# Gallicchio-Lab/openmm_agbnp_plugin

Hardware: AMD Instinct MI355X
Metric: AGBNP1 force-eval-limited ns/day (1 fs step), thrombin 1dwc, independent replicas (higher is better)
Workload: dtype f64

## Files before the change

### openmm_agbnp_plugin_amd/AGBNPplugin.py

```python
import ctypes as C

import numpy as np

from . import _lib


class OpenMMException(Exception):
    """Same role as OpenMM::OpenMMException in the reference: every API error surfaces as this type."""


def _md_unit_system():
    for name in ("openmm.unit", "simtk.unit"):
        try:
            module = __import__(name, fromlist=["md_unit_system"])
            return module.md_unit_system
        except Exception:
            continue
    return "md_unit_system"


def _strip_units(value):
    if hasattr(value, "value_in_unit_system"):
        return float(value.value_in_unit_system(_md_unit_system()))
    return float(value)
# ... 183 lines not shown
        if _lib.load().agbnp_hip_poll(self._h, C.byref(done), C.byref(bad)) != _lib.OK:
            raise OpenMMException("agbnp_hip_poll: no pinned status memory")
        return int(done.value), int(bad.value)

    def wait_verdict(self, evaluations=0, timeout=10.0):
        self._need()
        done, bad = C.c_int(0), C.c_int(0)
        rc = _lib.load().agbnp_hip_wait_verdict(self._h, int(evaluations), float(timeout), C.byref(done), C.byref(bad))
        if rc == _lib.ERR_TIMEOUT:
            raise OpenMMException(f"agbnp_hip_wait_verdict: timed out after {timeout} s with {int(done.value)} evaluation(s) judged")
        if rc != _lib.OK:
            raise OpenMMException("agbnp_hip_wait_verdict: no pinned status memory")
        return int(done.value), int(bad.value)

    def withheld(self):
        self._need()
        lib = _lib.load()
        n = lib.agbnp_hip_withheld_evaluations(self._h, None, 0)
        idx = np.full(max(n, 1), -1, dtype=np.int32)
        lib.agbnp_hip_withheld_evaluations(self._h, _ip(idx), n)
        return [int(k) for k in idx if k >= 0]

    def generation(self):
        self._need()
        return int(_lib.load().agbnp_hip_generation(self._h))

    def copyParametersToContext(self, force):
        self._need()
        r, g, a, q, h = force._arrays()
        rc = _lib.load().agbnp_hip_update_parameters(self._h, len(r), _dp(r), _dp(g), _dp(a), _dp(q), _ip(h))
        if rc != _lib.OK:
            raise OpenMMException(_lib.last_error(self._h))

    SCALARS = dict(e_vol1=0, e_vol2=1, e_atom=2, e_gb_pair=3, max_subtree_nodes=4, total_nodes=5, variant=6, max_local_atoms=7, forests=8, rows_on=9, row_builds=10, pack_level=11, pack_age=12, row_slice=13, pack_plans=14, overflow_kinds=15, launches=16, healed_forests=17)
    VECTORS = dict(selfvol_vdw=0, born=1, scale=2, selfvol_large=3, subtree_nodes=4, subtree_atoms=5)

    def scalar(self, name):
        self._need()
        v = C.c_double(0)
        rc = _lib.load().agbnp_hip_get_scalar(self._h, self.SCALARS[name], C.byref(v))
        if rc != _lib.OK:
            raise OpenMMException(_lib.last_error(self._h))
        return v.value

    def vector(self, name):
        self._need()
        out = np.zeros(self.numParticles)
        rc = _lib.load().agbnp_hip_get_vector(self._h, self.VECTORS[name], _dp(out))
        if rc != _lib.OK:
            raise OpenMMException(_lib.last_error(self._h))
        return out

    def tables(self):
        self._need()
        lib = _lib.load()
        ni, nj = C.c_int(0), C.c_int(0)
        lib.agbnp_hip_get_table_sizes(self._h, C.byref(ni), C.byref(nj))
        y = np.zeros(ni.value * nj.value * 16)
        y2 = np.zeros_like(y)
        ti = np.zeros(self.numParticles, dtype=np.int32)
        tj = np.zeros(self.numParticles, dtype=np.int32)
        lib.agbnp_hip_get_tables(self._h, _dp(y), _dp(y2), _ip(ti), _ip(tj))
        return dict(y=y.reshape(ni.value, nj.value, 16), y2=y2.reshape(ni.value, nj.value, 16), type_screened=ti, type_screener=tj)

    def set_diagnostics(self, enabled):
        self._need()
        _lib.load().agbnp_hip_set_diagnostics(self._h, 1 if enabled else 0)
# ... 70 lines not shown
```

### openmm_agbnp_plugin_amd/csrc/engine.hip

```cpp
#include <hip/hip_runtime.h>

#include <algorithm>
#include <atomic>
#include <chrono>
#include <cmath>
#include <cstdio>
#include <cstdlib>
#include <cstring>
#include <string>
#include <vector>

#include "../../include/agbnp_hip.h"
#include "adapter_kernels.h"
#include "agbnp_common.h"
#include "i4_tables.h"
#include "pair_kernels.h"
#include "tree_kernels.h"

namespace agbnp {
size_t tree_variant_lds_bytes(int variant);
size_t tree_variant_scratch_bytes(int variant);
int tree_variant_node_cap(int variant);
int tree_variant_atom_cap(int variant);
int tree_variant_wgs_per_cu(int variant);
// ... 369 lines not shown
  {
    void* dev = nullptr;
    P.host_status = (c->h_status && hipHostGetDevicePointer(&dev, c->h_status, 0) == hipSuccess) ? static_cast<volatile int*>(dev) : nullptr;
  }
  P.born_part = c->d_born_part.p;
  P.born = c->d_born.p;
  P.born_fp = c->d_born_fp.p;
  P.brw = c->d_brw.p;
  P.e_atom = c->d_e_atom.p;
  const size_t row = (size_t)c->n;
  P.gb_fx = c->d_gbf.p;
  P.gb_fy = c->d_gbf.p + c->n;
  P.gb_fz = c->d_gbf.p + 2 * (size_t)c->n;
  P.gb_items = c->d_gb_items.p;
  P.gb_items_count = (int)c->d_gb_items.count;
  P.db_fx = c->d_dbf.p;
  P.db_fy = c->d_dbf.p + row;
  P.db_fz = c->d_dbf.p + 2 * row;
  P.db_wu = c->d_dbf.p + 3 * row;
  P.egb_part = c->d_egb_part.p;
  {
    const bool wanted = c->rows_policy != 0;
    const bool gb_rows_possible = P.fast && c->d_nlg.p != nullptr && getenv("AGBNP_HIP_NO_GB_ROWS") == nullptr;
    P.rows_on = c->rows_capable && !c->rows_disabled && c->version == 1 && !P.det && (!P.single || gb_rows_possible) && wanted ? 1 : 0;
    P.gb_rows = P.rows_on && gb_rows_possible ? 1 : 0;
    const double reach = sqrt(P.range2) + c->skin, gb_reach = c->cutoff + c->skin;
    P.nl_build2 = reach * reach;
    P.nlg_build2 = gb_reach * gb_reach;
    P.nlg = c->d_nlg.p;
    P.nlg_count = c->d_nlg_count.p;
    P.nlg_stride = c->nlg_stride;
    P.nl_items = c->d_nl_items.p;
    P.nl_nitems = c->d_nl_nitems.p;
    P.nl_items_cap = c->nl_items_cap;
    {
      auto cap = [&](double radius, double density, int parts, int stride) {
        const double r = radius + 0.3, most = c->row_fill * density * (4.0 / 3.0) * M_PI * r * r * r / parts * c->row_boost;
        return std::max(256, (int)std::min(most + 255.0, 1e9) / 256 * 256);
      };
      P.nlh_cap = std::min(cap(reach, 52.0, kBornParts, c->nlh_stride), std::max(c->nlh_stride, 1));
      P.nla_cap = std::min(cap(reach, 105.0, kChainParts, c->nla_stride), std::max(c->nla_stride, 1));
      P.nlg_cap = std::min(cap(gb_reach, 105.0, kGbParts, c->nlg_stride), std::max(c->nlg_stride, 1));
    }
    if (P.gb_rows) {
      P.egb_part = c->d_egb_rows.p;
      P.egb_parts = (int)c->d_egb_rows.count;
    } else {
      P.egb_part = c->d_egb_part.p;
      P.egb_parts = (int)c->d_egb_part.count;
    }
    const double move = c->row_move >= 0.0 ? std::min(c->row_move, 0.5 * c->skin) : 0.5 * c->skin;
    P.nl_move2 = move * move;
    P.nl_flag = c->d_nl_flag.p;
    P.row_target = c->row_slice > 0 ? 0 : 2 * c->cus;
    P.nl_ref = c->d_nl_ref.p;
    P.hperm = c->d_hperm.p;
    P.aperm = c->d_aperm.p;
    P.hperm_n = (int)c->d_hperm.count;
    P.aperm_n = (int)c->d_aperm.count;
    P.nlh = c->d_nlh.p;
    P.nla = c->d_nla.p;
    P.nlh_count = c->d_nlh_count.p;
    P.nla_count = c->d_nla_count.p;
    P.nlh_stride = c->nlh_stride;
    P.nla_stride = c->nla_stride;
    P.bslice = c->d_bslice.p;
// ... 122 lines not shown
  if (getenv("AGBNP_HIP_ROW_STRIDE")) {
    c->nlh_stride = c->nla_stride = std::max(128, atoi(getenv("AGBNP_HIP_ROW_STRIDE")));
    if (c->nlg_stride) c->nlg_stride = c->nlh_stride;
  }
  const size_t born_lists = (size_t)((n + kRowGroup - 1) / kRowGroup) * kBornParts, chain_lists = (size_t)((nh + kRowGroup - 1) / kRowGroup) * kChainParts;
  HIP_TRY(c, c->d_nlh.alloc(born_lists * c->nlh_stride));
  HIP_TRY(c, c->d_nla.alloc(chain_lists * c->nla_stride));
  HIP_TRY(c, hipMemset(c->d_nlh.p, 0, sizeof(unsigned) * born_lists * c->nlh_stride));
  HIP_TRY(c, hipMemset(c->d_nla.p, 0, sizeof(unsigned) * chain_lists * c->nla_stride));
  {
    std::vector<unsigned> bs((n + kRowGroup - 1) / kRowGroup, 0u), cs((nh + kRowGroup - 1) / kRowGroup, 0u);
    for (int a = 0; a < n; a++) bs[a / kRowGroup] |= (unsigned)c->lut.type_screened[a] << (8 * (a % kRowGroup));
    for (int h = 0; h < nh; h++) cs[h / kRowGroup] |= (unsigned)c->lut.type_screener[c->h2a[h]] << (8 * (h % kRowGroup));
    HIP_TRY(c, c->d_bslice.upload(bs));
    HIP_TRY(c, c->d_cslice.upload(cs));
  }
  if (c->nlg_stride > 0) {
    const size_t gb_lists = (size_t)((n + kRowGroup - 1) / kRowGroup) * kGbParts;
    HIP_TRY(c, c->d_nlg.alloc(gb_lists * c->nlg_stride));
    HIP_TRY(c, hipMemset(c->d_nlg.p, 0, sizeof(unsigned) * gb_lists * c->nlg_stride));
    HIP_TRY(c, c->d_nlg_count.alloc(gb_lists));
    HIP_TRY(c, hipMemset(c->d_nlg_count.p, 0, sizeof(int) * gb_lists));
    const size_t waves = (gb_lists + 7) / 8 * 8 * (size_t)((c->nlg_stride + 255) / 256);
    HIP_TRY(c, c->d_egb_rows.alloc(waves));
    HIP_TRY(c, hipMemset(c->d_egb_rows.p, 0, sizeof(double) * waves));
  }
  {
    const size_t gb_lists = c->nlg_stride > 0 ? (size_t)((n + kRowGroup - 1) / kRowGroup) * kGbParts : 0;
    const size_t most = std::max(std::max(born_lists * ((c->nlh_stride + 255) / 256), chain_lists * ((c->nla_stride + 255) / 256)),
                                 gb_lists * ((c->nlg_stride + 255) / 256));
    c->nl_items_cap = (int)std::min<size_t>(most + 8, 1u << 30);
    HIP_TRY(c, c->d_nl_items.alloc((size_t)6 * c->nl_items_cap));
    HIP_TRY(c, hipMemset(c->d_nl_items.p, 0, sizeof(unsigned) * 6 * (size_t)c->nl_items_cap));
    HIP_TRY(c, c->d_nl_nitems.alloc(6));
    HIP_TRY(c, hipMemset(c->d_nl_nitems.p, 0, sizeof(int) * 6));
  }
  HIP_TRY(c, c->d_nlh_count.alloc(born_lists));
  HIP_TRY(c, c->d_nla_count.alloc(chain_lists));
  HIP_TRY(c, hipMemset(c->d_nlh_count.p, 0, sizeof(int) * born_lists));
  HIP_TRY(c, hipMemset(c->d_nla_count.p, 0, sizeof(int) * chain_lists));
  const std::vector<int> flag = {1, 0, c->row_slice > 0 ? std::min(std::max(c->row_slice, kRowSlice), kRowSliceMax) / 64 * 64 : kRowSlice, 0};
  HIP_TRY(c, c->d_nl_flag.upload(flag));
  HIP_TRY(c, c->d_nl_ref.alloc(3 * (size_t)n));
  HIP_TRY(c, hipMemset(c->d_nl_ref.p, 0xff, sizeof(double) * 3 * (size_t)n));
  HIP_TRY(c, c->d_bw.alloc(n));
  HIP_TRY(c, c->d_rec_h.alloc(nh));
  HIP_TRY(c, c->d_hrow.alloc(nh));
  HIP_TRY(c, c->d_grec.alloc(n));
  HIP_TRY(c, c->d_hrec.alloc(nh));
  HIP_TRY(c, hipMemset(c->d_hrec.p, 0, sizeof(double4) * nh));
  HIP_TRY(c, hipMemset(c->d_bw.p, 0, sizeof(double) * n));
  HIP_TRY(c, hipMemset(c->d_grec.p, 0, sizeof(double4) * n));
  const int nti = c->lut.nscreened, ntj = c->lut.nscreener, ni = kI4Nodes - 1;
  const size_t tab = (size_t)nti * ntj * ni;
  const double dr = kI4MaxA / (kI4Nodes - 1);
  std::vector<double2> pw(4 * tab);
  for (int ti = 0; ti < nti; ti++)
    for (int tj = 0; tj < ntj; tj++)
      for (int k = 0; k < ni; k++) {
        const size_t o = ((size_t)ti * ntj + tj) * kI4Nodes + k;
        const double y0 = c->lut.y[o], y1 = c->lut.y[o + 1], z0 = c->lut.y2[o] * dr * dr / 6.0, z1 = c->lut.y2[o + 1] * dr * dr / 6.0;
        const double2 ca = make_double2(y0, (y1 - y0) - std::fma(2.0, z0, z1)), cb = make_double2(3.0 * z0, z1 - z0);
        const size_t by_screened = ((size_t)ti * ntj + tj) * ni + k, by_screener = ((size_t)tj * nti + ti) * ni + k;
        pw[by_screened] = ca;
        pw[tab + by_screened] = cb;
        pw[2 * tab + by_screener] = ca;
        pw[3 * tab + by_screener] = cb;
      }
// ... 625 lines not shown
  if (c->lazy_evals) {
    HIP_TRY(c, hipSetDevice(c->device));
    const int rc_ = catch_up(c);
    if (rc_ != AGBNP_HIP_OK) return rc_;
  }
  if (which == 15) {
    const int* s = c->last_status;
    *value = (s[kStatStickyNode] ? 1 : 0) | (s[kStatStickyAtom] ? 2 : 0) | (s[kStatStickyPack] ? 4 : 0) | (s[kStatStickyRow] ? 8 : 0) |
             (s[kStatStickyOrder] ? 16 : 0) | (s[kStatStickyForest] << 5) | (s[kStatStickySplit] << 8);
    return AGBNP_HIP_OK;
  }
  if (which == 17) {
    *value = c->last_status[kStatStickyHealed];
    return AGBNP_HIP_OK;
  }
  if (!c->have_results) return c->fail(AGBNP_HIP_ERR_INVALID_ARGUMENT, "no completed evaluation yet");
  switch (which) {
    case 0: *value = c->last_components[0]; break;
    case 1: *value = c->last_components[1]; break;
    case 2: *value = c->last_components[2]; break;
    case 3: *value = c->last_components[3]; break;
    case 4: *value = c->last_status[kStatMaxNodes]; break;
    case 5: *value = c->last_status[kStatTotalNodes]; break;
    case 6: *value = c->variant; break;
    case 7: *value = c->last_status[kStatMaxAtoms]; break;
    case 8: *value = c->last_status[kStatForests]; break;
    case 9: *value = c->P.rows_on; break;
    case 10: *value = c->last_rows[1]; break;
    case 13: *value = c->last_rows[2]; break;
    case 11: *value = c->last_pack[0]; break;
    case 12: *value = c->last_pack[1]; break;
    case 14: *value = c->last_pack[3]; break;
    case 16: *value = c->version == 1 ? (c->five_active ? 5 : 6) : (c->five_active ? 2 : 3); break;
    default: return c->fail(AGBNP_HIP_ERR_INVALID_ARGUMENT, "unknown scalar id");
  }
  return AGBNP_HIP_OK;
}

int agbnp_hip_get_vector(agbnp_hip_context* c, int which, double* out) {
  if (!c || !out) return AGBNP_HIP_ERR_INVALID_ARGUMENT;
  if (c->lazy_evals) {
    HIP_TRY(c, hipSetDevice(c->device));
    const int rc_ = catch_up(c);
    if (rc_ != AGBNP_HIP_OK) return rc_;
  }
  if (!c->have_results) return c->fail(AGBNP_HIP_ERR_INVALID_ARGUMENT, "no completed evaluation yet");
  HIP_TRY(c, hipSetDevice(c->device));
  const int n = c->n, nh = c->nh;
  std::vector<double> tmp(std::max(n, std::max(nh, 1)));
  auto heavy_to_atoms = [&](const double* dsrc, size_t stride, size_t word, double scale_by_inv_vol) -> int {
    std::vector<double> raw((size_t)std::max(nh, 1) * stride);
    HIP_TRY(c, hipMemcpy(raw.data(), dsrc, sizeof(double) * raw.size(), hipMemcpyDeviceToHost));
    for (int i = 0; i < n; i++) out[i] = 0.0;
    for (int h = 0; h < nh; h++) {
      double v = raw[(size_t)h * stride + word];
      if (scale_by_inv_vol != 0.0) v /= (4. * M_PI * pow(c->r_vdw[c->h2a[h]], 3) / 3.);
      out[c->h2a[h]] = v;
    }
    return AGBNP_HIP_OK;
  };
  switch (which) {
    case 0: return heavy_to_atoms(c->hrow(kHvSvVdw), 1, 0, 0.0);
    case 1:
      if (c->version != 1) return c->fail(AGBNP_HIP_ERR_INVALID_ARGUMENT, "Born radii exist for version 1 only");
      HIP_TRY(c, hipMemcpy(out, c->d_born.p, sizeof(double) * n, hipMemcpyDeviceToHost));
      return AGBNP_HIP_OK;
// ... 224 lines not shown
```

### openmm_agbnp_plugin_amd/csrc/pair_kernels.h

```cpp
#pragma once
#include <hip/hip_runtime.h>

#include <vector>

#include "agbnp_common.h"

namespace agbnp {

struct OpenmmTargets {
  unsigned long long* force_fixed = nullptr;
  int padded = 0;
  const int* ctx_slot = nullptr;
  void* energy_buffer = nullptr;
  int energy_is_double = 1, energy_slot = 0;
};

struct OpenmmSource {
  const void* posq = nullptr;
  const float4* correction = nullptr;
  int is_double = 0;
  const int* atom_index = nullptr;
  const int* hslot = nullptr;
};

// ... 74 lines not shown
  double* born_part;
  double *born, *born_fp, *brw, *e_atom;
  double *gb_fx, *gb_fy, *gb_fz;
  const int* gb_items;
  int gb_items_count;
  const int* db_items;
  int db_items_count;
  double *db_fx, *db_fy, *db_fz, *db_wu;
  double* egb_part;
  int egb_parts;
  int rows_on;
  double nl_build2;
  double nl_move2;
  int row_target;
  int* nl_flag;
  double* nl_ref;
  const unsigned* hperm;
  const unsigned* aperm;
  int hperm_n, aperm_n;
  unsigned* nlh;
  int* nlh_count;
  int nlh_stride;
  unsigned* nla;
  int* nla_count;
  int nla_stride;
  int gb_rows;
  unsigned* nlg;
  int* nlg_count;
  int nlg_stride;
  double nlg_build2;
  unsigned* nl_items;
  int* nl_nitems;
  int nl_items_cap;
  int nlh_cap, nla_cap, nlg_cap;
  double4* rec_h;
  double4* hrow;
  double* bw;
  double4* grec;
  double4* hrec;
  const unsigned *bslice, *cslice;
  const double2 *pw_a, *pw_b;
  const double2 *pwt_a, *pwt_b;
};
__device__ __forceinline__ void rebase_for_parity(PairArgs& P, int after_role) {
  if (P.five != 2) return;
  const int par = (P.epoch[0] + after_role) & 1;
  const size_t toff = (size_t)par * P.table_doubles, noff = (size_t)(1 - par) * P.table_doubles;
  P.next_hv = P.hx + noff;
  P.next_sizes = P.sizes + (size_t)(1 - par) * P.sizes_stride;
  P.next_estatus = P.estatus + 16 * (1 - par);
  P.hx += toff, P.hy += toff, P.hz += toff;
  P.gx += toff, P.gy += toff, P.gz += toff;
  P.sv_vdw += toff, P.sv_large += toff;
  P.sizes += (size_t)par * P.sizes_stride;
  P.estatus += 16 * par;
}

constexpr int kRowGroup = 4;
constexpr int kRowSlice = 256, kRowWaves = 8;
#ifndef AGBNP_GB_ROW_WAVES
#define AGBNP_GB_ROW_WAVES 4
#endif
constexpr int kGbRowWaves = AGBNP_GB_ROW_WAVES;
constexpr int row_waves(int kind) { return kind == 2 ? kGbRowWaves : kRowWaves; }
constexpr int kRowSliceMax = 512;
constexpr int kChainParts = 4;
// ... 30 lines not shown
```

### openmm_agbnp_plugin_amd/csrc/pair_kernels.hip

```cpp
#include <hip/hip_runtime.h>

#include <algorithm>

#include "agbnp_common.h"
#include "device_math.h"
#include "pair_kernels.h"
#include "prep_role.h"

namespace agbnp {

#ifdef AGBNP_PAIR_STAMPS
constexpr int kPairLogSlots = 4096;
__device__ unsigned long long g_pair_log[3][kPairLogSlots][12];
#define PAIR_STAMP(kern, idx)                                                                                        \
  do {                                                                                                               \
    if (threadIdx.x == 0 && blockIdx.x < kPairLogSlots) g_pair_log[kern][blockIdx.x][idx] = wall_clock64();          \
  } while (0)
#define PAIR_STAMP_WAIT(kern, idx, what)                                                                            \
  do {                                                                                                               \
    asm volatile("s_waitcnt " what ::: "memory");                                                                    \
    PAIR_STAMP(kern, idx);                                                                                           \
  } while (0)
#define PAIR_STAMP_WHERE(kern, item)                                                                                 \
  do {                                                                                                               \
// ... 1011 lines not shown
  S.red[wave][0][lane] = kf * (double)fx.x;
  S.red[wave][1][lane] = kf * (double)fy.x;
  S.red[wave][2][lane] = kf * (double)fz.x;
  S.red[wave][3][lane] = (double)ys.x;
  S.red[wave][4][lane] = kf * (double)fx.y;
  S.red[wave][5][lane] = kf * (double)fy.y;
  S.red[wave][6][lane] = kf * (double)fz.y;
  S.red[wave][7][lane] = (double)ys.y;
  S.red[wave][8][jslot] = kf * (double)fxj;
  S.red[wave][9][jslot] = kf * (double)fyj;
  S.red[wave][10][jslot] = kf * (double)fzj;
  S.red[wave][11][jslot] = (double)yj;
  const double e = wave_sum((double)e2.x + (double)e2.y);
  if (lane == 0) s_e[wave] = e;
  __syncthreads();
  double* __restrict__ row = gb_rows + (size_t)wave * n;
  auto fold = [&](int r) { return (S.red[0][r][lane] + S.red[1][r][lane]) + (S.red[2][r][lane] + S.red[3][r][lane]); };
  const int ia = 64 * I0 + lane, ic = ia + 64, j = 64 * J + lane;
  const bool det = P.det != 0;
  const double qs = wave == 3 ? kQSum : kQGrad;
  if (ia < n) hbm_add(wave == 3 ? &P.ys[ysa] : &row[ia], quantize(fold(wave), qs, det));
  if (ic < n) hbm_add(wave == 3 ? &P.ys[ysc] : &row[ic], quantize(fold(4 + wave), qs, det));
  if (j < n) hbm_add(wave == 3 ? &P.ys[ysj] : &row[j], quantize(fold(8 + wave), qs, det));
  if (threadIdx.x == 0) egb_out[0] = 2.0 * kDielFactor * ((s_e[0] + s_e[1]) + (s_e[2] + s_e[3]));
}

template <bool kCut, bool kSingle, bool kFar, bool kMasks = false>
__global__ __launch_bounds__(256) void k_gb_tiles(int n, const int* __restrict__ items, const double4* __restrict__ aposq,
                                                  const double* __restrict__ born_part, const double* __restrict__ inv_rvdw,
                                                  const double* __restrict__ alpha, double* __restrict__ born,
                                                  double* __restrict__ born_fp, double* __restrict__ brw,
                                                  double* __restrict__ e_atom, double* __restrict__ gb_rows,
                                                  double* __restrict__ egb_part, PairArgs P) {
  if (kMasks && (int)blockIdx.x > P.gb_items_count) {
    if (((P.estatus[kStatOrderStale] & 2) | P.estatus[kStatMaskAging]) == 0) return;
    return neighbor_tile(P, (int)blockIdx.x - 1 - P.gb_items_count, true);
  }
  __shared__ __align__(16) char s_area[sizeof(StripSums)];
  static_assert(sizeof(StripSums) >= sizeof(TileSums) && sizeof(TileSums) >= kRoleScratchBytes, "the packing workgroup borrows the tile area");
  static_assert(sizeof(StripSums) >= sizeof(double2) * (3 * 128 + 6 * 64), "strip records fit the area of the sums");
  __shared__ double s_e[4];
  __shared__ int s_bmax[4];
  if (blockIdx.x == 0) {
    PAIR_STAMP(1, 0);
    rebase_for_parity(P, 0);
    packing_role<true>(P, s_area, (int)sizeof(StripSums));
    PAIR_STAMP(1, 3);
    return;
  }
  static_assert(sizeof(TileSums) >= sizeof(double2) * (3 * 128 + 3 * 64), "records fit the area of the sums");
  double2* const s_xy = reinterpret_cast<double2*>(s_area);
  double2* const s_zq = s_xy + 128;
  double2* const s_bb = s_zq + 128;
  double2* const s_ixy = s_bb + 128;
  double2* const s_izq = s_ixy + 64;
  double2* const s_ibc = s_izq + 64;
  const int lane = threadIdx.x & 63, wave = threadIdx.x >> 6;
  __builtin_amdgcn_s_setprio(3);
  const int item = items[blockIdx.x - 1];
  const int I = item & 0xfff, J = (item >> 12) & 0xfff;
  PAIR_STAMP(1, 0);
  if (item & kGbStripFlag) {
    if (kSingle) return gb_strip_f32<kCut>(n, I, J, aposq, born_part, inv_rvdw, gb_rows, egb_part + (blockIdx.x - 1), P, s_area, s_e);
    return gb_strip<kCut, kFar>(n, I, J, aposq, born_part, inv_rvdw, gb_rows, egb_part + (blockIdx.x - 1), P, s_area, s_e, s_bmax);
  }
  const bool diag = I == J;
  if (kCut && !diag) {
    double gap2 = 0.0;
    for (int d = 0; d < 3; d++) {
      const double g = fmax(0.0, fmax(P.abox[6 * J + d] - P.abox[6 * I + 3 + d], P.abox[6 * I + d] - P.abox[6 * J + 3 + d]));
      gap2 += g * g;
    }
    if (gap2 >= P.gb_cut2) {
      if (threadIdx.x == 0) egb_part[blockIdx.x - 1] = 0.0;
      return;
    }
  }
  PAIR_STAMP_WHERE(1, item);
  const int ysi = P.a2s[min(64 * I + lane, n - 1)], ysj = P.a2s[min(64 * J + lane, n - 1)];
  double beta_i = 0.0, beta_j = 0.0;
  if (P.rows_on && wave == 3) {
    const int ki = min(64 * I + lane, n - 1), kj = min(64 * J + lane, n - 1);
    const double ri = inv_rvdw[ki], rj = inv_rvdw[kj], pi = born_part[ki], pj = born_part[kj];
    beta_i = bw_beta(born_radius(ri, pi));
    beta_j = bw_beta(born_radius(rj, pj));
  }
  if (wave < 2) {
    const int a = 64 * (wave == 0 ? J : I) + lane;
    const bool va = a < n;
    const int ac = va ? a : n - 1;
    const double4 pa = aposq[ac];
    const BornRadius bra = born_radius(inv_rvdw[ac], born_part[ac]);
    const double qa = va ? pa.w : 0.0;
    if (wave == 0) {
      s_xy[lane] = s_xy[lane + 64] = make_double2(pa.x, pa.y);
      s_zq[lane] = s_zq[lane + 64] = make_double2(pa.z, qa);
      s_bb[lane] = s_bb[lane + 64] = make_double2(bra.br, bra.inv_br);
    } else {
      s_ixy[lane] = make_double2(pa.x, pa.y);
      s_izq[lane] = make_double2(pa.z, qa);
      s_ibc[lane] = make_double2(bra.br, (-0.25 * 1.4426950408889634074) * bra.inv_br);
      if (diag && va) {
        const double bh = bra.br + kHBRadius, bh3 = bh * bh * bh, al = alpha[a];
        const double brw_a = -(1. / (4. * kPi)) * 3. * al * bra.br * bra.br * bra.fp / (bh3 * bh);
        born[a] = bra.br;
        born_fp[a] = bra.fp;
        e_atom[a] = al / bh3 + kDielFactor * pa.w * pa.w * bra.inv_br;
// ... 38 lines not shown
    fyj = fma(-dy, mw, fyj);
    fzj = fma(-dz, mw, fzj);
    const double yt = fma(0.25, d2, bb) * (et * s3);
    yi += yt;
    yj_acc += yt;
    fxj = rot1(fxj);
    fyj = rot1(fyj);
    fzj = rot1(fzj);
    yj_acc = rot1(yj_acc);
  }
  const double kf = -2.0 * kDielFactor;
  __builtin_amdgcn_s_setprio(3);
  __syncthreads();
  PAIR_STAMP(1, 2);
  TileSums& s_sums = *reinterpret_cast<TileSums*>(s_area);
  {
    const double vi4[4] = {kf * fxi, kf * fyi, kf * fzi, yi}, vj4[4] = {kf * fxj, kf * fyj, kf * fzj, yj_acc};
    tile_sums_store(s_sums, wave, lane, (lane + start + nsteps) & 63, vi4, vj4);
  }
  e = wave_sum(e);
  if (lane == 0) s_e[wave] = e;
  __syncthreads();
  double* __restrict__ row = gb_rows + (size_t)wave * n;
  const int i = 64 * I + lane, j = 64 * J + lane;
  const bool det = P.det != 0;
  const double qs = wave == 3 ? kQSum : kQGrad;
  if (P.rows_on && wave == 3) {
    if (i < n) hbm_add(&P.bw[i], beta_i * tile_sums_fold(s_sums, 3, lane));
    if (j < n) hbm_add(&P.bw[j], beta_j * tile_sums_fold(s_sums, 7, lane));
  } else {
    if (i < n) hbm_add(wave == 3 ? &P.ys[ysi] : &row[i], quantize(tile_sums_fold(s_sums, wave, lane), qs, det));
    if (j < n) hbm_add(wave == 3 ? &P.ys[ysj] : &row[j], quantize(tile_sums_fold(s_sums, 4 + wave, lane), qs, det));
  }
  if (threadIdx.x == 0) egb_part[blockIdx.x - 1] = 2.0 * kDielFactor * ((s_e[0] + s_e[1]) + (s_e[2] + s_e[3]));
  PAIR_STAMP(1, 3);
}

template <bool kBoth>
__device__ __forceinline__ void born_walk(double& sum_i, double& sum_j, const double2* __restrict__ s_lut,
                                          const double2* __restrict__ jxy, const double2* __restrict__ jzs,
                                          const double* __restrict__ jty, double xi, double yi, double zi, double si, int row,
                                          int tsr, int nsteps, int masked_step, bool vi, bool lower, int ntj, double range2) {
#pragma unroll 4
  for (int k = 0; k < nsteps; k++) {
    const double2 xy = jxy[k], zs = jzs[k];
    const double ty = jty[k];
    const double dx = xy.x - xi, dy = xy.y - yi, dz = zs.x - zi;
    const double d2 = fma(dz, dz, fma(dy, dy, dx * dx));
    const int tj = __double2loint(ty);
    if (d2 < range2 && vi && __double2hiint(ty) >= 0 && (k != masked_step || lower)) {
      const double d = d2 * rsqrt_pos(d2);
      sum_j = fma(si, spline_value(s_lut, ((tj & 0xffff) * ntj + tsr) * kLutStride, d), sum_j);
      if (kBoth) sum_i = fma(zs.y, spline_value(s_lut, (row + (tj >> 16)) * kLutStride, d), sum_i);
    }
    sum_j = rot1(sum_j);
  }
}

__global__ __launch_bounds__(256) void k_born_tiles(int nh, int nhb, int ntj, int lut_entries, const int* __restrict__ items,
                                                   const int* __restrict__ pslot, const double* __restrict__ pbox,
                                                   const double4* __restrict__ prec, const double* __restrict__ sv_vdw,
                                                   const double* __restrict__ inv_vol_h, const double2* __restrict__ lut,
                                                   double* __restrict__ born_part, double range2, int det, int cull_first) {
  extern __shared__ double2 s_lut[];
  __shared__ double2 s_xy[128], s_zs[128];
  __shared__ double s_ty[128];
  __shared__ double2 s_ixy[64], s_izs[64];
// ... 216 lines not shown
  const double qs = wave == 3 ? kQSum : kQGrad;
  if (vi) hbm_add(&row[wave == 3 ? 64 * I + lane : ai], quantize(tile_sums_fold(s_sums, wave, lane), qs, det));
  if (aj >= 0 && (both || wave < 3)) hbm_add(&row[wave == 3 ? 64 * J + lane : aj], quantize(tile_sums_fold(s_sums, 4 + wave, lane), qs, det));
  PAIR_STAMP(2, 3);
}

template <int KIND, bool SINGLE = false, bool MASKS = false, bool DEVPAR = false>
__global__ __launch_bounds__(64 * row_waves(KIND), KIND == kGbRows ? 4 : 6) void k_rows(PairArgs P, double* __restrict__ energy_out, double* __restrict__ components, int role_bytes) {
  extern __shared__ double2 s_dyn[];

  int blk = blockIdx.x;
  if (MASKS && KIND == kBornRows && blk >= role_bytes) {
    if (threadIdx.x >= 256) return;
    if (DEVPAR) rebase_for_parity(P, 0);
    if (((P.estatus[kStatOrderStale] & 2) | P.estatus[kStatMaskAging]) == 0) return;
    return neighbor_tile(P, blk - role_bytes, true);
  }
  if (KIND == kChainRows) {
    if (blk < 2 && threadIdx.x >= 256) return;
    if (blk == 0) return energy_role<DEVPAR>(P, 1, energy_out, components, reinterpret_cast<char*>(s_dyn));
    if (blk == 1) return dealing_role(P, reinterpret_cast<char*>(s_dyn), role_bytes);
    blk -= 2;
  }
  if (KIND == kGbRows) {
    if (blk == 0) {
      static_assert(kGbRowWaves >= 4, "the bookkeeping role is written for 256 lanes");
      if (threadIdx.x >= 256) return;
      PAIR_STAMP(1, 0);
      rebase_for_parity(P, 0);
      packing_role<false>(P, reinterpret_cast<char*>(s_dyn), role_bytes);
      PAIR_STAMP(1, 3);
      return;
    }
    blk -= 1;
  }
  __shared__ int s_busy;
  rows_workgroup<KIND, row_waves(KIND), SINGLE, MASKS && DEVPAR>(P, blk, s_dyn, &s_busy);
}


__global__ __launch_bounds__(256) void k_outputs(PairArgs P, int version, double* __restrict__ force_out,
                                                 double* __restrict__ energy_out, double* __restrict__ components, int role_bytes,
                                                 int mask_from) {
  extern __shared__ char s_role[];
  int blk = blockIdx.x;
  if (mask_from >= 0 && blk >= mask_from) {
    if (((P.estatus[kStatOrderStale] & 2) | P.estatus[kStatMaskAging]) == 0) return;
    return neighbor_tile(P, blk - mask_from, true);
  }
  rebase_for_parity(P, 1);
  if (version != 1) {
    if (blk == 0) return energy_role(P, version, energy_out, components, s_role);
    if (blk == 1) {
      packing_role<true>(P, s_role, role_bytes);
      __threadfence();
      __syncthreads();
      return dealing_role(P, s_role, role_bytes);
    }
    blk -= 2;
  }
  const int t = threadIdx.x;
  const int i = blk * 256 + t;
  if (P.rows_on && i == 0) {
    rows_close_evaluation(P.nl_flag, P.nl_nitems, P.row_target, P.gb_rows != 0);
  }
  if (i >= P.n) return;
  double fx = 0, fy = 0, fz = 0;
// ... 64 lines not shown
  const size_t lds = (size_t)P.lut_entries * sizeof(double2);
  if (lds > 32 * 1024) {
    hipError_t e = hipFuncSetAttribute(reinterpret_cast<const void*>(k_born_tiles), hipFuncAttributeMaxDynamicSharedMemorySize, (int)lds);
    if (e != hipSuccess) return e;
    e = hipFuncSetAttribute(reinterpret_cast<const void*>(k_dborn_tiles), hipFuncAttributeMaxDynamicSharedMemorySize, (int)(lds + 3 * 64 * sizeof(double2)));
    if (e != hipSuccess) return e;
  }
  if (P.rows_on) {
    auto gb = P.fast ? k_gb_tiles<true, false, false> : (P.gb_far ? k_gb_tiles<false, false, true> : k_gb_tiles<false, false, false>);
    const int born_groups = (P.n + kRowGroup - 1) / kRowGroup, chain_groups = (P.nh + kRowGroup - 1) / kRowGroup;
    auto walk_blocks = [](int lists, int cap) { return (lists + kRowWaves - 1) / kRowWaves * ((cap + kRowSlice - 1) / kRowSlice); };
    const int born_blocks = walk_blocks(born_groups * kBornParts, P.nlh_cap), chain_blocks = walk_blocks(chain_groups * kChainParts, P.nla_cap);
    const int gb_blocks = (born_groups * kGbParts + kGbRowWaves - 1) / kGbRowWaves * ((P.nlg_cap + kRowSlice - 1) / kRowSlice);
    const int build_blocks = (chain_groups * kChainParts + (P.gb_rows ? born_groups * kGbParts : 0) + kRowWaves - 1) / kRowWaves;
    const size_t table_lds = (size_t)2 * P.nti * P.ntj * kRowIntervals * sizeof(double2);
    const size_t born_lds = table_lds, chain_lds = std::max(table_lds, sizeof(TileSums));
    AGBNP_MARK(kKBornRows);
    if (P.single && P.five)
      hipLaunchKernelGGL((k_rows<kBornRows, true, true>), dim3(born_blocks + build_blocks + P.nb_tiles), dim3(64 * kRowWaves), born_lds, st, P, (double*)nullptr,
                         (double*)nullptr, born_blocks + build_blocks);
    else if (P.single)
      hipLaunchKernelGGL((k_rows<kBornRows, true>), dim3(born_blocks + build_blocks), dim3(64 * kRowWaves), born_lds, st, P, (double*)nullptr, (double*)nullptr, 0);
    else if (P.five == 2)
      hipLaunchKernelGGL((k_rows<kBornRows, false, true, true>), dim3(born_blocks + build_blocks + P.nb_tiles), dim3(64 * kRowWaves), born_lds, st, P,
                         (double*)nullptr, (double*)nullptr, born_blocks + build_blocks);
    else if (P.five)
      hipLaunchKernelGGL((k_rows<kBornRows, false, true>), dim3(born_blocks + build_blocks + P.nb_tiles), dim3(64 * kRowWaves), born_lds, st, P, (double*)nullptr,
                         (double*)nullptr, born_blocks + build_blocks);
    else
      hipLaunchKernelGGL(k_rows<kBornRows>, dim3(born_blocks + build_blocks), dim3(64 * kRowWaves), born_lds, st, P, (double*)nullptr, (double*)nullptr, 0);
    AGBNP_CHECK_LAUNCH();
    if (P.gb_rows) {
      AGBNP_MARK(kKGbRows);
      hipLaunchKernelGGL(k_rows<kGbRows>, dim3(1 + gb_blocks), dim3(64 * kGbRowWaves), sizeof(StripSums), st, P, (double*)nullptr, (double*)nullptr, (int)sizeof(StripSums));
    } else {
      AGBNP_MARK(kKGbTiles);
      hipLaunchKernelGGL(gb, dim3(P.gb_items_count + 1), dim3(256), 0, st, P.n, P.gb_items, (const double4*)P.aposq,
                         (const double*)P.born_part, P.inv_rvdw, P.alpha, P.born, P.born_fp, P.brw, P.e_atom, P.gb_fx, P.egb_part, P);
    }
    AGBNP_CHECK_LAUNCH();
    AGBNP_MARK(kKDbornRows);
    if (P.single)
      hipLaunchKernelGGL((k_rows<kChainRows, true>), dim3(2 + chain_blocks), dim3(64 * kRowWaves), chain_lds, st, P, energy_out, components, (int)chain_lds);
    else if (P.five == 2)
      hipLaunchKernelGGL((k_rows<kChainRows, false, false, true>), dim3(2 + chain_blocks), dim3(64 * kRowWaves), chain_lds, st, P, energy_out, components, (int)chain_lds);
    else
      hipLaunchKernelGGL(k_rows<kChainRows>, dim3(2 + chain_blocks), dim3(64 * kRowWaves), chain_lds, st, P, energy_out, components, (int)chain_lds);
    AGBNP_CHECK_LAUNCH();
    return hipSuccess;
  }
  AGBNP_MARK(kKBornTiles);
  if (P.db_items_count > 0)
    hipLaunchKernelGGL(k_born_tiles, dim3(P.db_items_count), dim3(256), lds, st, P.nh, P.nhb, P.ntj, P.lut_entries, P.db_items, P.pslot,
                       (const double*)P.pbox, (const double4*)P.prec, (const double*)P.sv_vdw, P.inv_vol_h, P.lut, P.born_part, P.range2, P.det, P.cull_first);
  AGBNP_CHECK_LAUNCH();
  AGBNP_MARK(kKGbTiles);
  auto gb = P.fast ? (P.single ? k_gb_tiles<true, true, false> : k_gb_tiles<true, false, false>)
                   : (P.gb_far ? k_gb_tiles<false, false, true> : k_gb_tiles<false, false, false>);
  if (P.five)
    gb = P.fast ? (P.single ? k_gb_tiles<true, true, false, true> : k_gb_tiles<true, false, false, true>)
                : (P.gb_far ? k_gb_tiles<false, false, true, true> : k_gb_tiles<false, false, false, true>);
  hipLaunchKernelGGL(gb, dim3(P.gb_items_count + 1 + (P.five ? P.nb_tiles : 0)), dim3(256), 0, st, P.n, P.gb_items, (const double4*)P.aposq,
                     (const double*)P.born_part, P.inv_rvdw, P.alpha, P.born, P.born_fp, P.brw, P.e_atom, P.gb_fx, P.egb_part, P);
  AGBNP_CHECK_LAUNCH();
  AGBNP_MARK(kKDbornTiles);
  const size_t db_lds = std::max(lds + 3 * 64 * sizeof(double2), sizeof(TileSums));
  hipLaunchKernelGGL(k_dborn_tiles, dim3(P.db_items_count + 2), dim3(256), db_lds, st, P.n, P.nhb, P.ntj, P.lut_entries, P.db_items, P.pslot,
                     (const double*)P.pbox, (const double4*)P.prec, (const double4*)P.srec, (const double*)P.ys, (const double*)P.sv_vdw,
                     P.inv_vol_h, P.nh, P.lut, P.db_fx, P, energy_out, components, (int)db_lds);
  AGBNP_CHECK_LAUNCH();
// ... 25 lines not shown
```

### openmm_agbnp_plugin_amd/csrc/row_kernels.h

```cpp
#pragma once
#include <hip/hip_runtime.h>

#include "agbnp_common.h"
#include "device_math.h"
#include "pair_kernels.h"

#ifndef PAIR_STAMP
#define PAIR_STAMP(kern, idx)
#define PAIR_STAMP_WAIT(kern, idx, what)
#define PAIR_STAMP_WHERE(kern, item)
#endif
#ifndef PAIR_STAMP_HW
#define PAIR_STAMP_HW(kern)
#endif
#ifndef ROWS_LOG_COUNTS
#define ROWS_LOG_COUNTS(kern, todo, nsteps)
#endif

namespace agbnp {

__device__ __forceinline__ void hbm_add(double* p, double v) {
#ifdef AGBNP_TIMING_NO_ATOMICS
  if (v == 1.2345e300) *p = v;
  return;
// ... 107 lines not shown
  (void)gb_rows;
  const int wgs = (items + kRowWaves - 1) / kRowWaves, rs = nl_flag[2];
  if (wgs > row_target && wgs <= 2 * row_target && rs < kRowSliceMax) {
    nl_flag[2] = max(rs, kRowSlice) + 64;
    nl_flag[0] = 1;
  }
}

struct RowLists {
  unsigned* list;
  int* count;
  int stride, cap, groups, parts;
};
template <int KIND>
__device__ __forceinline__ RowLists row_lists(const PairArgs& P) {
  RowLists L;
  L.list = KIND == kBornRows ? P.nlh : KIND == kChainRows ? P.nla : P.nlg;
  L.count = KIND == kBornRows ? P.nlh_count : KIND == kChainRows ? P.nla_count : P.nlg_count;
  L.stride = KIND == kBornRows ? P.nlh_stride : KIND == kChainRows ? P.nla_stride : P.nlg_stride;
  L.cap = KIND == kBornRows ? P.nlh_cap : KIND == kChainRows ? P.nla_cap : P.nlg_cap;
  L.groups = ((KIND == kChainRows ? P.nh : P.n) + kRowGroup - 1) / kRowGroup;
  L.parts = KIND == kBornRows ? kBornParts : KIND == kChainRows ? kChainParts : kGbParts;
  return L;
}
template <int KIND>
__device__ __forceinline__ void append_items(const PairArgs& P, int sub, int entries, bool at_least_one) {
  const int rs = row_slice_length(P);
  const int nsl = max((entries + rs - 1) / rs, at_least_one ? 1 : 0);
  if (nsl == 0) return;
  const int buf = (P.nl_flag[1] + 1) & 1;
  const int base = atomicAdd(&P.nl_nitems[2 * KIND + buf], nsl);
  unsigned* items = P.nl_items + (size_t)(2 * KIND + buf) * P.nl_items_cap;
  for (int sl = 0; sl < nsl && base + sl < P.nl_items_cap; sl++) items[base + sl] = (unsigned)sub | ((unsigned)sl << 24);
}

template <int KIND>
__device__ __forceinline__ void build_list(const PairArgs& P, int sub, int lane, int stale, int* estatus) {
  const RowLists L = row_lists<KIND>(P);
  if (sub >= L.groups * L.parts) return;
  if (!stale) {
    if (lane == 0 && L.count[sub] > L.cap) estatus[kStatRowOverflow] = 1;
    return;
  }
  const int g = sub / L.parts, part = sub - g * L.parts;
  const RowAtoms A = row_atoms<KIND>(P, g);
  const int cnt = row_build(A, P.aperm, P.aperm_n, part, L.parts, static_cast<const double4*>(P.aposq), KIND == kGbRows ? P.nlg_build2 : P.nl_build2,
                            L.list + (size_t)sub * L.stride, L.stride, lane);
  if (lane == 0) {
    L.count[sub] = cnt;
    if (cnt > L.cap) estatus[kStatRowOverflow] = 1;
    append_items<KIND>(P, sub, min(cnt, L.cap), KIND == kGbRows && part == 0);
  }
}

template <int KIND, int WAVES, bool SINGLE = false, bool PARITY = false>
__device__ __forceinline__ void rows_workgroup(const PairArgs& P, int blk, double2* s_dyn, int* s_busy_word) {
  static_assert(!SINGLE || KIND != kGbRows, "the GB rows choose their precision at run time (P.single)");
  constexpr int R = kRowGroup;
  static_assert(R == 4, "the butterfly below folds 16 sums");
  int& s_busy = *s_busy_word;
  const int lane = threadIdx.x & 63, wave = __builtin_amdgcn_readfirstlane(threadIdx.x >> 6);
  const RowLists L = row_lists<KIND>(P);
  const int NP = L.parts, stride = L.stride;
  const int nlists = L.groups * NP, lists_pad = (nlists + WAVES - 1) / WAVES * WAVES;
  const int stale = P.nl_flag[0];
  const int epoch_now = PARITY ? P.epoch[0] : 0;
// ... 349 lines not shown
```

Measured before the change: 887.7.

## Deal born and chain row items across waves by length to balance work

Adds two extra workgroups to the GB launch that histogram the born and chain row items by step count. They then reorder each list in a serpentine deal, so every wave in a row workgroup gets a similar total number of steps. The aim is to cut load imbalance and tail time in the following row kernels. The cost is two extra workgroups that read and rewrite the item lists, plus a few global counters that also back new diagnostic scalars.

```diff
diff --git a/openmm_agbnp_plugin_amd/AGBNPplugin.py b/openmm_agbnp_plugin_amd/AGBNPplugin.py
--- a/openmm_agbnp_plugin_amd/AGBNPplugin.py
+++ b/openmm_agbnp_plugin_amd/AGBNPplugin.py
@@ -239,7 +239,9 @@
         if rc != _lib.OK:
             raise OpenMMException(_lib.last_error(self._h))
 
-    SCALARS = dict(e_vol1=0, e_vol2=1, e_atom=2, e_gb_pair=3, max_subtree_nodes=4, total_nodes=5, variant=6, max_local_atoms=7, forests=8, rows_on=9, row_builds=10, pack_level=11, pack_age=12, row_slice=13, pack_plans=14, overflow_kinds=15, launches=16, healed_forests=17)
+    SCALARS = dict(e_vol1=0, e_vol2=1, e_atom=2, e_gb_pair=3, max_subtree_nodes=4, total_nodes=5, variant=6, max_local_atoms=7, forests=8, rows_on=9, row_builds=10, pack_level=11, pack_age=12, row_slice=13, pack_plans=14, overflow_kinds=15, launches=16, healed_forests=17,
+                   born_wg_steps_max_appended=18, born_wg_steps_max=19, born_wg_steps_mean=20,
+                   chain_wg_steps_max_appended=21, chain_wg_steps_max=22, chain_wg_steps_mean=23)
     VECTORS = dict(selfvol_vdw=0, born=1, scale=2, selfvol_large=3, subtree_nodes=4, subtree_atoms=5)
 
     def scalar(self, name):
diff --git a/openmm_agbnp_plugin_amd/csrc/engine.hip b/openmm_agbnp_plugin_amd/csrc/engine.hip
--- a/openmm_agbnp_plugin_amd/csrc/engine.hip
+++ b/openmm_agbnp_plugin_amd/csrc/engine.hip
@@ -425,6 +425,7 @@
     P.nlg_stride = c->nlg_stride;
     P.nl_items = c->d_nl_items.p;
     P.nl_nitems = c->d_nl_nitems.p;
+    P.nl_deal = c->d_nl_nitems.p ? c->d_nl_nitems.p + 6 : nullptr;
     P.nl_items_cap = c->nl_items_cap;
     {
       auto cap = [&](double radius, double density, int parts, int stride) {
@@ -613,8 +614,8 @@
     c->nl_items_cap = (int)std::min<size_t>(most + 8, 1u << 30);
     HIP_TRY(c, c->d_nl_items.alloc((size_t)6 * c->nl_items_cap));
     HIP_TRY(c, hipMemset(c->d_nl_items.p, 0, sizeof(unsigned) * 6 * (size_t)c->nl_items_cap));
-    HIP_TRY(c, c->d_nl_nitems.alloc(6));
-    HIP_TRY(c, hipMemset(c->d_nl_nitems.p, 0, sizeof(int) * 6));
+    HIP_TRY(c, c->d_nl_nitems.alloc(6 + 8));
+    HIP_TRY(c, hipMemset(c->d_nl_nitems.p, 0, sizeof(int) * (6 + 8)));
   }
   HIP_TRY(c, c->d_nlh_count.alloc(born_lists));
   HIP_TRY(c, c->d_nla_count.alloc(chain_lists));
@@ -1306,6 +1307,16 @@
     case 12: *value = c->last_pack[1]; break;
     case 14: *value = c->last_pack[3]; break;
     case 16: *value = c->version == 1 ? (c->five_active ? 5 : 6) : (c->five_active ? 2 : 3); break;
+    case 18: case 19: case 20: case 21: case 22: case 23: {
+      if (!c->d_nl_nitems.p) return c->fail(AGBNP_HIP_ERR_INVALID_ARGUMENT, "no row form in this context");
+      int deal[8];
+      HIP_TRY(c, hipSetDevice(c->device));
+      HIP_TRY(c, hipMemcpy(deal, c->d_nl_nitems.p + 6, sizeof(deal), hipMemcpyDeviceToHost));
+      const int* d = deal + 4 * ((which - 18) / 3);
+      const int what = (which - 18) % 3;
+      *value = what == 0 ? d[0] : what == 1 ? d[1] : (d[3] > 0 ? (double)d[2] / d[3] : 0.0);
+      break;
+    }
     default: return c->fail(AGBNP_HIP_ERR_INVALID_ARGUMENT, "unknown scalar id");
   }
   return AGBNP_HIP_OK;
diff --git a/openmm_agbnp_plugin_amd/csrc/pair_kernels.h b/openmm_agbnp_plugin_amd/csrc/pair_kernels.h
--- a/openmm_agbnp_plugin_amd/csrc/pair_kernels.h
+++ b/openmm_agbnp_plugin_amd/csrc/pair_kernels.h
@@ -130,6 +130,7 @@
   unsigned* nl_items;
   int* nl_nitems;
   int nl_items_cap;
+  int* nl_deal;
   int nlh_cap, nla_cap, nlg_cap;
   double4* rec_h;
   double4* hrow;
diff --git a/openmm_agbnp_plugin_amd/csrc/pair_kernels.hip b/openmm_agbnp_plugin_amd/csrc/pair_kernels.hip
--- a/openmm_agbnp_plugin_amd/csrc/pair_kernels.hip
+++ b/openmm_agbnp_plugin_amd/csrc/pair_kernels.hip
@@ -1067,9 +1067,10 @@
                                                   double* __restrict__ born_fp, double* __restrict__ brw,
                                                   double* __restrict__ e_atom, double* __restrict__ gb_rows,
                                                   double* __restrict__ egb_part, PairArgs P) {
-  if (kMasks && (int)blockIdx.x > P.gb_items_count) {
+  const int roles = P.rows_on ? 3 : 1;
+  if (kMasks && (int)blockIdx.x >= roles + P.gb_items_count) {
     if (((P.estatus[kStatOrderStale] & 2) | P.estatus[kStatMaskAging]) == 0) return;
-    return neighbor_tile(P, (int)blockIdx.x - 1 - P.gb_items_count, true);
+    return neighbor_tile(P, (int)blockIdx.x - roles - P.gb_items_count, true);
   }
   __shared__ __align__(16) char s_area[sizeof(StripSums)];
   static_assert(sizeof(StripSums) >= sizeof(TileSums) && sizeof(TileSums) >= kRoleScratchBytes, "the packing workgroup borrows the tile area");
@@ -1083,6 +1084,12 @@
     PAIR_STAMP(1, 3);
     return;
   }
+  if ((int)blockIdx.x < roles) {
+    static_assert(sizeof(StripSums) >= sizeof(int) * 32, "the deal's counts fit the tile area");
+    if (blockIdx.x == 1) return row_deal_role<kBornRows>(P, reinterpret_cast<int*>(s_area));
+    return row_deal_role<kChainRows>(P, reinterpret_cast<int*>(s_area));
+  }
+  const int tile = (int)blockIdx.x - roles;
   static_assert(sizeof(TileSums) >= sizeof(double2) * (3 * 128 + 3 * 64), "records fit the area of the sums");
   double2* const s_xy = reinterpret_cast<double2*>(s_area);
   double2* const s_zq = s_xy + 128;
@@ -1092,12 +1099,12 @@
   double2* const s_ibc = s_izq + 64;
   const int lane = threadIdx.x & 63, wave = threadIdx.x >> 6;
   __builtin_amdgcn_s_setprio(3);
-  const int item = items[blockIdx.x - 1];
+  const int item = items[tile];
   const int I = item & 0xfff, J = (item >> 12) & 0xfff;
   PAIR_STAMP(1, 0);
   if (item & kGbStripFlag) {
-    if (kSingle) return gb_strip_f32<kCut>(n, I, J, aposq, born_part, inv_rvdw, gb_rows, egb_part + (blockIdx.x - 1), P, s_area, s_e);
-    return gb_strip<kCut, kFar>(n, I, J, aposq, born_part, inv_rvdw, gb_rows, egb_part + (blockIdx.x - 1), P, s_area, s_e, s_bmax);
+    if (kSingle) return gb_strip_f32<kCut>(n, I, J, aposq, born_part, inv_rvdw, gb_rows, egb_part + tile, P, s_area, s_e);
+    return gb_strip<kCut, kFar>(n, I, J, aposq, born_part, inv_rvdw, gb_rows, egb_part + tile, P, s_area, s_e, s_bmax);
   }
   const bool diag = I == J;
   if (kCut && !diag) {
@@ -1107,7 +1114,7 @@
       gap2 += g * g;
     }
     if (gap2 >= P.gb_cut2) {
-      if (threadIdx.x == 0) egb_part[blockIdx.x - 1] = 0.0;
+      if (threadIdx.x == 0) egb_part[tile] = 0.0;
       return;
     }
   }
@@ -1212,7 +1219,7 @@
     if (i < n) hbm_add(wave == 3 ? &P.ys[ysi] : &row[i], quantize(tile_sums_fold(s_sums, wave, lane), qs, det));
     if (j < n) hbm_add(wave == 3 ? &P.ys[ysj] : &row[j], quantize(tile_sums_fold(s_sums, 4 + wave, lane), qs, det));
   }
-  if (threadIdx.x == 0) egb_part[blockIdx.x - 1] = 2.0 * kDielFactor * ((s_e[0] + s_e[1]) + (s_e[2] + s_e[3]));
+  if (threadIdx.x == 0) egb_part[tile] = 2.0 * kDielFactor * ((s_e[0] + s_e[1]) + (s_e[2] + s_e[3]));
   PAIR_STAMP(1, 3);
 }
 
@@ -1495,7 +1502,9 @@
       PAIR_STAMP(1, 3);
       return;
     }
-    blk -= 1;
+    if (blk == 1) return row_deal_role<kBornRows>(P, reinterpret_cast<int*>(s_dyn));
+    if (blk == 2) return row_deal_role<kChainRows>(P, reinterpret_cast<int*>(s_dyn));
+    blk -= 3;
   }
   __shared__ int s_busy;
   rows_workgroup<KIND, row_waves(KIND), SINGLE, MASKS && DEVPAR>(P, blk, s_dyn, &s_busy);
@@ -1626,10 +1635,10 @@
     AGBNP_CHECK_LAUNCH();
     if (P.gb_rows) {
       AGBNP_MARK(kKGbRows);
-      hipLaunchKernelGGL(k_rows<kGbRows>, dim3(1 + gb_blocks), dim3(64 * kGbRowWaves), sizeof(StripSums), st, P, (double*)nullptr, (double*)nullptr, (int)sizeof(StripSums));
+      hipLaunchKernelGGL(k_rows<kGbRows>, dim3(3 + gb_blocks), dim3(64 * kGbRowWaves), sizeof(StripSums), st, P, (double*)nullptr, (double*)nullptr, (int)sizeof(StripSums));
     } else {
       AGBNP_MARK(kKGbTiles);
-      hipLaunchKernelGGL(gb, dim3(P.gb_items_count + 1), dim3(256), 0, st, P.n, P.gb_items, (const double4*)P.aposq,
+      hipLaunchKernelGGL(gb, dim3(P.gb_items_count + 3), dim3(256), 0, st, P.n, P.gb_items, (const double4*)P.aposq,
                          (const double*)P.born_part, P.inv_rvdw, P.alpha, P.born, P.born_fp, P.brw, P.e_atom, P.gb_fx, P.egb_part, P);
     }
     AGBNP_CHECK_LAUNCH();
diff --git a/openmm_agbnp_plugin_amd/csrc/row_kernels.h b/openmm_agbnp_plugin_amd/csrc/row_kernels.h
--- a/openmm_agbnp_plugin_amd/csrc/row_kernels.h
+++ b/openmm_agbnp_plugin_amd/csrc/row_kernels.h
@@ -163,6 +163,111 @@
   const int base = atomicAdd(&P.nl_nitems[2 * KIND + buf], nsl);
   unsigned* items = P.nl_items + (size_t)(2 * KIND + buf) * P.nl_items_cap;
   for (int sl = 0; sl < nsl && base + sl < P.nl_items_cap; sl++) items[base + sl] = (unsigned)sub | ((unsigned)sl << 24);
+}
+
+__device__ __forceinline__ int item_steps(unsigned it, const int* count, int cap, int rs) {
+  const int sl = (int)(it >> 24), len = min(count[it & 0xffffffu], cap);
+  return min(max((min(len - sl * rs, rs) + 63) >> 6, 0), kRowSliceMax / 64);
+}
+__device__ __forceinline__ int deal_position(int k, int w, int last) {
+  int r, pos, width;
+  if (k < last * w) {
+    r = k / w, pos = k - r * w, width = w;
+  } else {
+    const int kk = k - last * w;
+    r = last + kk / (w - 1), pos = kk - (r - last) * (w - 1), width = w - 1;
+  }
+  const int g = (r & 1) ? width - 1 - pos : pos;
+  const int wave = (g == w - 1 && last < kRowWaves) ? r : (r < kRowWaves / 2 ? r : kRowWaves + kRowWaves / 2 - 1 - r);
+  return g * kRowWaves + wave;
+}
+template <int KIND>
+__device__ void row_deal_role(const PairArgs& P, int* s_deal) {
+  static_assert(KIND == kBornRows || KIND == kChainRows, "the GB rows walk their items in the launch that would deal them");
+  static_assert(kRowWaves == 8 && kRowSliceMax / 64 == 8, "the deal is laid out for eight waves and up to eight steps");
+  constexpr int kB = kRowSliceMax / 64 + 1, kBatch = 8;
+  if (threadIdx.x >= 256 || !P.nl_flag[0]) return;
+  PAIR_STAMP(1, 0);
+  const int tid = threadIdx.x;
+  const int buf = (P.nl_flag[1] + 1) & 1;
+  const int n = min(P.nl_nitems[2 * KIND + buf], P.nl_items_cap);
+  unsigned* const items = P.nl_items + (size_t)(2 * KIND + buf) * P.nl_items_cap;
+  unsigned* const spare = P.nl_items + (size_t)(2 * KIND + (buf ^ 1)) * P.nl_items_cap;
+  const int* const count = KIND == kBornRows ? P.nlh_count : P.nla_count;
+  const int cap = KIND == kBornRows ? P.nlh_cap : P.nla_cap, rs = row_slice_length(P);
+  int* const hist = s_deal;
+  int* const start = s_deal + kB;
+  int* const cursor = s_deal + 2 * kB;
+  int* const most = s_deal + 3 * kB;
+  if (tid < kB) hist[tid] = 0;
+  if (tid < 2) most[tid] = 0;
+  __syncthreads();
+  for (int b0 = 0; b0 < n; b0 += 256 * kBatch) {
+    unsigned it[kBatch];
+    int len[kBatch];
+#pragma unroll
+    for (int j = 0; j < kBatch; j++) it[j] = items[min(b0 + 256 * j + tid, max(n - 1, 0))];
+#pragma unroll
+    for (int j = 0; j < kBatch; j++) len[j] = item_steps(it[j], count, cap, rs);
+#pragma unroll
+    for (int j = 0; j < kBatch; j++) {
+      const bool in = b0 + 256 * j + tid < n;
+      if (in) atomicAdd(&hist[len[j]], 1);
+      int t = in ? len[j] : 0;
+      t += __shfl_xor(t, 1, 64), t += __shfl_xor(t, 2, 64), t += __shfl_xor(t, 4, 64);
+      if ((tid & 7) == 0) atomicMax(&most[0], t);
+    }
+  }
+  __syncthreads();
+  if (tid == 0) {
+    int at = 0, total = 0;
+    for (int b = kB - 1; b >= 0; b--) start[b] = cursor[b] = at, at += hist[b], total += b * hist[b];
+    P.nl_deal[4 * KIND + 2] = total;
+    P.nl_deal[4 * KIND + 3] = (n + kRowWaves - 1) / kRowWaves;
+  }
+  __syncthreads();
+  const int w = (n + kRowWaves - 1) / kRowWaves, last = n - kRowWaves * (w - 1);
+  for (int g = tid; g < w; g += 256) {
+    int t = 0;
+    for (int r = 0; r < kRowWaves; r++) {
+      int k;
+      if (r < last) {
+        k = r * w + ((r & 1) ? w - 1 - g : g);
+      } else {
+        if (g == w - 1) break;
+        k = last * w + (r - last) * (w - 1) + ((r & 1) ? w - 2 - g : g);
+      }
+      int b = kB - 1;
+      while (b > 0 && k >= start[b] + hist[b]) b--;
+      t += b;
+    }
+    atomicMax(&most[1], t);
+  }
+  for (int b0 = 0; b0 < n; b0 += 256 * kBatch) {
+    unsigned it[kBatch];
+    int len[kBatch];
+#pragma unroll
+    for (int j = 0; j < kBatch; j++) it[j] = items[min(b0 + 256 * j + tid, n - 1)];
+#pragma unroll
+    for (int j = 0; j < kBatch; j++) len[j] = item_steps(it[j], count, cap, rs);
+#pragma unroll
+    for (int j = 0; j < kBatch; j++)
+      if (b0 + 256 * j + tid < n) spare[deal_position(atomicAdd(&cursor[len[j]], 1), w, last)] = it[j];
+  }
+  __builtin_amdgcn_fence(__ATOMIC_RELEASE, "agent");
+  __syncthreads();
+  __builtin_amdgcn_fence(__ATOMIC_ACQUIRE, "agent");
+  for (int b0 = 0; b0 < n; b0 += 256 * kBatch) {
+    unsigned it[kBatch];
+#pragma unroll
+    for (int j = 0; j < kBatch; j++) it[j] = spare[min(b0 + 256 * j + tid, n - 1)];
+#pragma unroll
+    for (int j = 0; j < kBatch; j++)
+      if (b0 + 256 * j + tid < n) items[b0 + 256 * j + tid] = it[j];
+  }
+  __syncthreads();
+  if (tid == 0) P.nl_deal[4 * KIND] = most[0], P.nl_deal[4 * KIND + 1] = most[1];
+  PAIR_STAMP(1, 3);
 }
 
 template <int KIND>
```

New measurement: 892.6 (median of 6 runs). About the same (+0.5%).
